# AndrewCullacino/handwritten-chinese-ocr-samples

Hardware: AMD Instinct MI355X
Metric: text-lines/sec (1x128x2000 synth) greedy decode (higher is better)
Workload: dtype f16 (f32 accumulate); 1 GPU; BASELINE configs[1]: 64 x 1x128x2000 uint8 lines, random-init hctr checkpoint (C=7358), forward + greedy CTC decode, labels to host; global_lines=64, lines_per_gpu=64, width=2000, classes=7358, checkpoint=random, parallelism=batch-shard x1

## Files before the change

### handwritten-chinese-ocr-samples_amd/csrc/kernels.hip

```cpp
#include "kernels.h"

#include <algorithm>
#include <cstdlib>

namespace hctr {

typedef _Float16 f16x8 __attribute__((ext_vector_type(8)));
typedef float f32x4 __attribute__((ext_vector_type(4)));
typedef float f32x2 __attribute__((ext_vector_type(2)));
typedef _Float16 f16x2 __attribute__((ext_vector_type(2)));
typedef uint32_t u32x4 __attribute__((ext_vector_type(4)));
typedef void __attribute__((address_space(3))) * lptr_t;

__device__ __forceinline__ void glds16_asm(const char* gsrc, char* lds_dst) {
    const uint32_t lds = (uint32_t)(uintptr_t)((lptr_t)lds_dst);
    uint32_t keep;
    asm volatile("s_mov_b32 %0, m0\n\ts_mov_b32 m0, %2\n\ts_nop 0\n\tglobal_load_lds_dwordx4 %1, off\n\ts_mov_b32 m0, %0"
                 : "=&s"(keep)
                 : "v"(gsrc), "s"(lds)
                 : "memory");
}

template <int CTRL>
__device__ __forceinline__ float dpp_f32(float v) {
    return __builtin_bit_cast(float, __builtin_amdgcn_update_dpp(0, __builtin_bit_cast(int, v), CTRL, 0xF, 0xF, true));
}

__device__ __forceinline__ bool np_gt(float a, float b) { return a > b || (a != a && b == b); }
__device__ __forceinline__ bool np_eq(float a, float b) { return a == b || (a != a && b != b); }

__device__ __forceinline__ void glds16_asm_s(const char* sbase, uint32_t voff, char* lds_dst) {
    const uint32_t lds = (uint32_t)(uintptr_t)((lptr_t)lds_dst);
    uint32_t keep;
    asm volatile("s_mov_b32 %0, m0\n\ts_mov_b32 m0, %3\n\ts_nop 0\n\tglobal_load_lds_dwordx4 %1, %2\n\ts_mov_b32 m0, %0"
                 : "=&s"(keep)
                 : "v"(voff), "s"(sbase), "s"(lds)
                 : "memory");
}

__device__ __forceinline__ void glds16x4_asm_s(const char* s0, const char* s1, const char* s2, const char* s3, uint32_t voff,
                                               char* d0, char* d1, char* d2, char* d3) {
    const uint32_t l0 = (uint32_t)(uintptr_t)((lptr_t)d0), l1 = (uint32_t)(uintptr_t)((lptr_t)d1);
    const uint32_t l2 = (uint32_t)(uintptr_t)((lptr_t)d2), l3 = (uint32_t)(uintptr_t)((lptr_t)d3);
    uint32_t keep;
    asm volatile("s_mov_b32 %0, m0\n\t"
                 "s_mov_b32 m0, %6\n\ts_nop 0\n\tglobal_load_lds_dwordx4 %1, %2\n\t"
                 "s_mov_b32 m0, %7\n\ts_nop 0\n\tglobal_load_lds_dwordx4 %1, %3\n\t"
                 "s_mov_b32 m0, %8\n\ts_nop 0\n\tglobal_load_lds_dwordx4 %1, %4\n\t"
                 "s_mov_b32 m0, %9\n\ts_nop 0\n\tglobal_load_lds_dwordx4 %1, %5\n\t"
                 "s_mov_b32 m0, %0"
                 : "=&s"(keep)
                 : "v"(voff), "s"(s0), "s"(s1), "s"(s2), "s"(s3), "s"(l0), "s"(l1), "s"(l2), "s"(l3)
                 : "memory");
}

template <int LSTRIDE>
__device__ __forceinline__ void glds16x4v_asm_s(const char* sbase, uint32_t v0, uint32_t v1, uint32_t v2, uint32_t v3, char* d0) {
    const uint32_t l0 = (uint32_t)(uintptr_t)((lptr_t)d0);
    uint32_t keep;
    asm volatile("s_mov_b32 %0, m0\n\t"
                 "s_mov_b32 m0, %6\n\ts_nop 0\n\tglobal_load_lds_dwordx4 %1, %5\n\t"
                 "s_add_u32 m0, m0, %7\n\ts_nop 0\n\tglobal_load_lds_dwordx4 %2, %5\n\t"
                 "s_add_u32 m0, m0, %7\n\ts_nop 0\n\tglobal_load_lds_dwordx4 %3, %5\n\t"
                 "s_add_u32 m0, m0, %7\n\ts_nop 0\n\tglobal_load_lds_dwordx4 %4, %5\n\t"
                 "s_mov_b32 m0, %0"
                 : "=&s"(keep)
                 : "v"(v0), "v"(v1), "v"(v2), "v"(v3), "s"(sbase), "s"(l0), "i"(LSTRIDE)
                 : "memory", "scc");
}

__device__ __forceinline__ constexpr int acc_cout_offset(int j) { return (j >> 2) * 64 + ((j >> 1) & 1) * 32 + (j & 1) * 4; }

constexpr float kSeScaleFloor = 1e-12f;

template <int WN, int WM, int JT, bool LINEAR, bool SPLIT, bool PRIVATE_RED = false, bool BIAS_DONE = false,
          bool RESID_IN_ACC = false>
__device__ __forceinline__ void conv_epilogue(const ConvArgs& a, f32x4 (&acc)[JT][4], char* smem, int tid, int lane,
                                              int wn, int wm, int n0, int mt, int img, int th, int tw, int hbase,
                                              int w0, unsigned long long* st = nullptr) {
    auto estamp = [&](int i) {
        if (st != nullptr) {
            __builtin_amdgcn_sched_barrier(0);
            if (tid == 0) st[i] = __builtin_amdgcn_s_memrealtime();
            __builtin_amdgcn_sched_barrier(0);
        }
    };
    constexpr int WC = JT * 16;
    constexpr int BN = WN * WC, BM = WM * 64;
    const int q = lane >> 4;
    const int c = lane & 15;
    const int cw0 = n0 + wn * WC + q * 8;
    auto co = [](int j) { return acc_cout_offset(j); };

    if (!BIAS_DONE) {
#pragma unroll
        for (int j = 0; j < JT; ++j) {
            const f32x4 b4 = *(const f32x4*)(a.bias + cw0 + co(j));
#pragma unroll
            for (int n = 0; n < 4; ++n)
#pragma unroll
                for (int i = 0; i < 4; ++i) acc[j][n][i] += b4[i];
        }
    }

    estamp(8);
    if (LINEAR && a.emit_cnt != nullptr) {
        static_assert(!LINEAR || WN == kLinearWN, "partials per n-tile");
        const int64_t part = (int64_t)((n0 / BN) * WN + wn) * a.M;
#pragma unroll
        for (int n = 0; n < 4; ++n) {
            const int64_t m = (int64_t)mt * BM + wm * 64 + n * 16 + c;
            const bool mv = m < a.M;
            const float vmin = mv ? a.row_thr[2 * m] : INFINITY;
            const float gmax = mv ? a.row_thr[2 * m + 1] : 0.f;
            double es = 0.0;
#pragma unroll
            for (int j = 0; j < JT; ++j)
#pragma unroll
                for (int i = 0; i < 4; ++i) {
                    const int cls = cw0 + co(j) + i;
                    const float v = acc[j][n][i];
                    if (cls < a.Cout) {
                        es += (double)expf(v - gmax);
                        if (v >= vmin) {
                            const int pos = atomicAdd(a.emit_cnt + m, 1);
                            if (pos < a.emit_cap) {
                                int32_t* e = a.emit_list + ((int64_t)m * a.emit_cap + pos) * 2;
                                e[0] = cls;
                                e[1] = __builtin_bit_cast(int32_t, v);
                            }
                        }
                    }
                }
            es += __shfl_xor(es, 16);
            es += __shfl_xor(es, 32);
            if (q == 0 && mv) a.esum[part + m] = es;
        }
        return;
    }
    if (LINEAR && a.amax_idx != nullptr) {
        static_assert(!LINEAR || WN == kLinearWN, "partials per n-tile");
        const int64_t part = (int64_t)((n0 / BN) * WN + wn) * a.M;
        const bool guard = a.amax_val2 != nullptr;
#pragma unroll
        for (int n = 0; n < 4; ++n) {
            float bv = -INFINITY, sv = -INFINITY, av = 0.f;
            int bi = 0x7fffffff;
            if (!guard) {
#pragma unroll
                for (int j = 0; j < JT; ++j)
#pragma unroll
                    for (int i = 0; i < 4; ++i) {
                        const int cls = cw0 + co(j) + i;
                        const float v = acc[j][n][i];
                        if (cls < a.Cout && np_gt(v, bv)) { bv = v; bi = cls; }
                    }
            } else {
#pragma unroll
                for (int j = 0; j < JT; ++j)
#pragma unroll
                    for (int i = 0; i < 4; ++i) {
                        const int cls = cw0 + co(j) + i;
                        const float v = acc[j][n][i];
                        if (cls < a.Cout) {
                            av = fmaxf(av, fabsf(v));
                            if (np_gt(v, bv)) { sv = bv; bv = v; bi = cls; }
                            else if (np_gt(v, sv)) sv = v;
                        }
                    }
            }
#pragma unroll
            for (int off = 16; off <= 32; off <<= 1) {
                const float ov = __shfl_xor(bv, off);
                const int oi = __shfl_xor(bi, off);
                const bool wins = np_gt(ov, bv) || (np_eq(ov, bv) && oi < bi);
                if (guard) {
                    const float osv = __shfl_xor(sv, off);
                    const float lose = wins ? bv : ov, keep2 = wins ? osv : sv;
                    sv = np_gt(lose, keep2) ? lose : keep2;
                    av = fmaxf(av, __shfl_xor(av, off));
                }
                if (wins) { bv = ov; bi = oi; }
            }
            const int64_t m = (int64_t)mt * BM + wm * 64 + n * 16 + c;
            if (q == 0 && m < a.M) {
                a.amax_val[part + m] = bv;
                a.amax_idx[part + m] = bi;
                if (guard) {
                    a.amax_val2[part + m] = sv;
                    a.amax_abs[part + m] = av;
                }
            }
            if (a.psum != nullptr) {
                float ps = 0.f;
#pragma unroll
                for (int j = 0; j < JT; ++j)
#pragma unroll
                    for (int i = 0; i < 4; ++i)
                        if (cw0 + co(j) + i < a.Cout) ps += expf(acc[j][n][i] - bv);
                ps += __shfl_xor(ps, 16);
                ps += __shfl_xor(ps, 32);
                if (q == 0 && m < a.M) {
                    a.psum[part + m] = ps;
                    if (cw0 == 0) a.blank_logit[m] = acc[0][n][0];
                }
            }
        }
        return;
    }
    if (LINEAR) {
        float* out = (float*)a.y;
#pragma unroll
        for (int n = 0; n < 4; ++n) {
            const int64_t m = (int64_t)mt * BM + wm * 64 + n * 16 + c;
            if (m < a.M) {
#pragma unroll
                for (int j = 0; j < JT; ++j)
                    *(f32x4*)(out + m * a.ldo + cw0 + co(j)) = acc[j][n];
            }
        }
        return;
    }

    const int w = w0 + c;
    const bool wvalid = w < a.W;
    half_t* out = (half_t*)a.y;
    const int64_t pix0 = a.out_off + img * a.out_sb + (int64_t)w * a.out_sw + cw0;

    if (SPLIT && !RESID_IN_ACC && a.se_scale != nullptr) {
        const float* sc = a.se_scale + (int64_t)img * a.Cout + cw0;
        if (w < a.out_wlimit) {
#pragma unroll
            for (int cb = 0; cb < JT / 4; ++cb)
#pragma unroll
                for (int n = 0; n < 4; ++n) {
                    const half_t* r = a.resid + pix0 + (int64_t)(hbase + n) * a.out_sh + cb * 64;
                    const f16x8 h0 = *(const f16x8*)r, h1 = *(const f16x8*)(r + 32);
                    const f16x8 l0 = *(const f16x8*)(r + a.Cout), l1 = *(const f16x8*)(r + a.Cout + 32);
#pragma unroll
                    for (int e = 0; e < 16; ++e) {
                        const float rv = e < 8 ? (float)h0[e] + (float)l0[e] : (float)h1[e - 8] + (float)l1[e - 8];
                        const float sv = sc[cb * 64 + (e >> 3) * 32 + (e & 7)];
                        acc[cb * 4 + (e >> 2)][n][e & 3] = fmaf(acc[cb * 4 + (e >> 2)][n][e & 3], sv, rv);
                    }
                }
        }
    } else if (RESID_IN_ACC) {
        const float* sc = a.se_scale + (int64_t)img * a.Cout + cw0;
#pragma unroll
        for (int j = 0; j < JT; ++j) {
            const f32x4 s4 = *(const f32x4*)(sc + co(j));
#pragma unroll
            for (int n = 0; n < 4; ++n)
#pragma unroll
                for (int i = 0; i < 4; ++i) acc[j][n][i] *= fmaxf(s4[i], kSeScaleFloor);
        }
    } else if (a.se_scale != nullptr) {
        const float* sc = a.se_scale + (int64_t)img * a.Cout + cw0;
        if (w < a.out_wlimit) {
            f16x8 rlo[JT / 4][4], rhi[JT / 4][4];
#pragma unroll
            for (int cb = 0; cb < JT / 4; ++cb)
#pragma unroll
                for (int n = 0; n < 4; ++n) {
                    const half_t* r = a.resid + pix0 + (int64_t)(hbase + n) * a.out_sh + cb * 64;
                    rlo[cb][n] = *(const f16x8*)r;
                    rhi[cb][n] = *(const f16x8*)(r + 32);
                }
#pragma unroll
            for (int j = 0; j < JT; ++j) {
                const f32x4 s4 = *(const f32x4*)(sc + co(j));
#pragma unroll
                for (int n = 0; n < 4; ++n)
#pragma unroll
                    for (int i = 0; i < 4; ++i) {
                        const int e = (j & 3) * 4 + i;
                        const float r = e < 8 ? (float)rlo[j >> 2][n][e] : (float)rhi[j >> 2][n][e - 8];
                        acc[j][n][i] = fmaf(acc[j][n][i], s4[i], r);
                    }
            }
        }
    }

    estamp(9);
    if (!SPLIT) {
        const _Float16 lo1 = a.relu ? (_Float16)0.f : (_Float16)(-INFINITY);
        const f16x2 lo2 = {lo1, lo1};
        const uint32_t keep = wvalid ? 0xffffffffu : 0u;
        uint32_t P[JT][4][2];
#pragma unroll
        for (int j = 0; j < JT; ++j)
#pragma unroll
            for (int n = 0; n < 4; ++n) {
                f32x4 v = acc[j][n];
                if (a.pool) {
                    const f32x4 u = acc[j][n | 1];
#pragma unroll
                    for (int i = 0; i < 4; ++i) v[i] = fmaxf(acc[j][n & ~1][i], u[i]);
                }
                f16x2 h0 = __builtin_convertvector((f32x2){v[0], v[1]}, f16x2);
                f16x2 h1 = __builtin_convertvector((f32x2){v[2], v[3]}, f16x2);
                h0 = __builtin_elementwise_max(h0, lo2);
                h1 = __builtin_elementwise_max(h1, lo2);
                P[j][n][0] = __builtin_bit_cast(uint32_t, h0) & keep;
                P[j][n][1] = __builtin_bit_cast(uint32_t, h1) & keep;
            }
        estamp(10);
        if (a.se_part != nullptr) {
            if (!PRIVATE_RED) {
                asm volatile("s_waitcnt vmcnt(0)" ::: "memory");
                __syncthreads();
            }
            float* red = (float*)smem;
            constexpr int NV = JT * 4;
            float vals[NV];
#pragma unroll
            for (int j = 0; j < JT; ++j)
#pragma unroll
                for (int i = 0; i < 4; ++i) {
                    float t[4];
#pragma unroll
                    for (int n = 0; n < 4; ++n)
                        t[n] = (float)__builtin_bit_cast(f16x2, P[j][n][i >> 1])[i & 1];
                    vals[j * 4 + i] = (t[0] + t[1]) + (t[2] + t[3]);
                }
            const bool e0 = ((c ^ (c >> 2)) & 1) != 0, e1 = (((c >> 1) ^ (c >> 2)) & 1) != 0;
            const bool e2 = (((c >> 2) ^ (c >> 3)) & 1) != 0, e3 = ((c >> 3) & 1) != 0;
            float r1[NV / 2], r2[NV / 4], r3[NV / 8], r4[NV / 16];
#pragma unroll
            for (int u = 0; u < NV / 2; ++u)
                r1[u] = (e0 ? vals[2 * u + 1] : vals[2 * u]) + dpp_f32<0xB1>(e0 ? vals[2 * u] : vals[2 * u + 1]);
#pragma unroll
            for (int u = 0; u < NV / 4; ++u)
                r2[u] = (e1 ? r1[2 * u + 1] : r1[2 * u]) + dpp_f32<0x4E>(e1 ? r1[2 * u] : r1[2 * u + 1]);
#pragma unroll
            for (int u = 0; u < NV / 8; ++u)
                r3[u] = (e2 ? r2[2 * u + 1] : r2[2 * u]) + dpp_f32<0x141>(e2 ? r2[2 * u] : r2[2 * u + 1]);
#pragma unroll
            for (int u = 0; u < NV / 16; ++u)
                r4[u] = (e3 ? r3[2 * u + 1] : r3[2 * u]) + dpp_f32<0x140>(e3 ? r3[2 * u] : r3[2 * u + 1]);
            const int vlow = (e3 ? 8 : 0) + (e2 ? 4 : 0) + (e1 ? 2 : 0) + (e0 ? 1 : 0);
#pragma unroll
            for (int u = 0; u < NV / 16; ++u) {
                const int v = 16 * u + vlow, j = v >> 2, i = v & 3;
                red[wm * BN + wn * WC + q * 8 + ((j >> 2) * 64 + ((j >> 1) & 1) * 32 + (j & 1) * 4) + i] = r4[u];
            }
            __syncthreads();
            if (tid < BN) {
                float sum = 0.f;
#pragma unroll
                for (int m = 0; m < WM; ++m) sum += red[m * BN + tid];
                const int64_t tile = (int64_t)img * (a.tilesH * a.tilesW) + th * a.tilesW + tw;
                if (n0 + tid < a.Cout) a.se_part[tile * a.Cout + n0 + tid] = sum;
            }
        }
        estamp(11);
        if (a.dbg & 256) {
            uint32_t t = 0;
#pragma unroll
            for (int j = 0; j < JT; ++j)
#pragma unroll
                for (int n = 0; n < 4; ++n) t += P[j][n][0] ^ P[j][n][1];
            if (t == 0x12345678u) out[0] = (half_t)1.f;
        } else if (w < a.out_wlimit) {
#pragma unroll
            for (int n = 0; n < 4; ++n) {
                if (a.pool && (n & 1)) continue;
                const int ho = a.pool ? ((hbase + n) >> 1) : (hbase + n);
                half_t* o = out + pix0 + (int64_t)ho * a.out_sh;
#pragma unroll
                for (int cb = 0; cb < JT / 4; ++cb) {
                    const int j0 = cb * 4;
                    *(u32x4*)(o + cb * 64) = (u32x4){P[j0][n][0], P[j0][n][1], P[j0 + 1][n][0], P[j0 + 1][n][1]};
                    *(u32x4*)(o + cb * 64 + 32) =
                        (u32x4){P[j0 + 2][n][0], P[j0 + 2][n][1], P[j0 + 3][n][0], P[j0 + 3][n][1]};
                }
            }
        }
        return;
    }
#pragma unroll
    for (int j = 0; j < JT; ++j)
#pragma unroll
        for (int n = 0; n < 4; ++n)
#pragma unroll
            for (int i = 0; i < 4; ++i) {
                float v = acc[j][n][i];
                if (a.pool && (n & 1) == 0) v = fmaxf(v, acc[j][n + 1][i]);
                if (a.relu) v = fmaxf(v, 0.f);
                if (!wvalid) v = 0.f;
                if (SPLIT) {
                    const half_t hi = (half_t)v;
                    v = a.drop_lo ? (float)hi : (float)hi + (float)(half_t)(v - (float)hi);
                } else {
                    v = (float)(half_t)v;
                }
                acc[j][n][i] = v;
            }

    estamp(10);
    if (a.se_part != nullptr) {
        if (!PRIVATE_RED) {
            asm volatile("s_waitcnt vmcnt(0)" ::: "memory");
            __syncthreads();
        }
        float* red = (float*)smem;
#pragma unroll
        for (int j = 0; j < JT; ++j)
#pragma unroll
            for (int i = 0; i < 4; ++i) {
                float s = (acc[j][0][i] + acc[j][1][i]) + (acc[j][2][i] + acc[j][3][i]);
                s += dpp_f32<0xB1>(s);
                s += dpp_f32<0x4E>(s);
                s += dpp_f32<0x141>(s);
                s += dpp_f32<0x140>(s);
                if (c == 0) red[wm * BN + wn * WC + q * 8 + co(j) + i] = s;
            }
        __syncthreads();
        if (tid < BN) {
            float s = 0.f;
#pragma unroll
            for (int m = 0; m < WM; ++m) s += red[m * BN + tid];
            const int64_t tile = (int64_t)img * (a.tilesH * a.tilesW) + th * a.tilesW + tw;
            if (n0 + tid < a.Cout) a.se_part[tile * a.Cout + n0 + tid] = s;
        }
    }

    estamp(11);
    if (a.dbg & 256) {
        float t = 0.f;
#pragma unroll
        for (int j = 0; j < JT; ++j)
#pragma unroll
            for (int n = 0; n < 4; ++n) t += acc[j][n][0] + acc[j][n][1] + acc[j][n][2] + acc[j][n][3];
        if (t == 123.456f) out[0] = (half_t)t;
    } else if (w < a.out_wlimit) {
#pragma unroll
        for (int n = 0; n < 4; ++n) {
            if (a.pool && (n & 1)) continue;
            const int ho = a.pool ? ((hbase + n) >> 1) : (hbase + n);
            half_t* o = out + pix0 + (int64_t)ho * a.out_sh;
#pragma unroll
            for (int cb = 0; cb < JT / 4; ++cb) {
                f16x8 lo, hi;
#pragma unroll
                for (int e = 0; e < 16; ++e) {
                    const half_t hv = (half_t)acc[cb * 4 + (e >> 2)][n][e & 3];
                    if (e < 8) lo[e] = hv; else hi[e - 8] = hv;
                }
                *(f16x8*)(o + cb * 64) = lo;
                *(f16x8*)(o + cb * 64 + 32) = hi;
                if (SPLIT) {
                    f16x8 l0, l1;
#pragma unroll
                    for (int e = 0; e < 16; ++e) {
                        const float v = acc[cb * 4 + (e >> 2)][n][e & 3];
                        const half_t lv = (half_t)(v - (float)(half_t)v);
                        if (e < 8) l0[e] = lv; else l1[e - 8] = lv;
                    }
                    *(f16x8*)(o + a.Cout + cb * 64) = l0;
                    *(f16x8*)(o + a.Cout + cb * 64 + 32) = l1;
                    *(f16x8*)(o + 2 * a.Cout + cb * 64) = lo;
                    *(f16x8*)(o + 2 * a.Cout + cb * 64 + 32) = hi;
                }
            }
        }
    }
}

template <int WN, int WM, int JT, int TAPS, bool LINEAR, bool PIPE, bool SPLIT>
__global__ __launch_bounds__(WN* WM * 64) void conv_mfma_kernel(const ConvArgs a) {
    constexpr int NT = WN * WM * 64;
    constexpr int WC = JT * 16;
    constexpr int BN = WN * WC, BM = WM * 64;
    constexpr int NIW = BN * 8 / NT;
    constexpr int NIX = BM * 8 / NT;
    constexpr int TILE_BYTES = (BN + BM) * 128;
    extern __shared__ __attribute__((aligned(16))) char smem[];

    const int tid = threadIdx.x;
    const int lane = tid & 63;
    const int wv = __builtin_amdgcn_readfirstlane(tid >> 6);
    const int wn = wv / WM, wm = wv % WM;

    const int total = a.mtiles * a.ntiles;
    int lin;
    {
        const int id = blockIdx.x, xcd = id & 7, s = id >> 3;
        const int q = total >> 3, r = total & 7;
        lin = (xcd < r ? xcd * (q + 1) : r * (q + 1) + (xcd - r) * q) + s;
    }
    const int nt = lin % a.ntiles;
    const int mt = lin / a.ntiles;
    const int n0 = nt * BN;

    int img = 0, th = 0, tw = 0;
    if (!LINEAR) {
        tw = mt % a.tilesW;
        const int t2 = mt / a.tilesW;
        th = t2 % a.tilesH;
        img = t2 / a.tilesH;
    }
    const int cin = a.Cin;

    const char* xbase;
    if (LINEAR) xbase = (const char*)(a.x + (int64_t)mt * BM * cin);
    else xbase = (const char*)(a.x + img * a.in_sb);
    const char* wbase = (const char*)(a.w + (int64_t)n0 * cin);
    uint32_t xoff[NIX], woff[NIW];
#pragma unroll
    for (int i = 0; i < NIX; ++i) {
        const int g = (wv * NIX + i) * 64 + lane;
        const int row = g >> 3, cp = (g & 7) ^ (row & 7);
        if (LINEAR) {
            int64_t rem = a.M - (int64_t)mt * BM;
            const int r = (int64_t)row < rem ? row : (int)rem - 1;
            xoff[i] = (uint32_t)r * (uint32_t)cin * 2u + cp * 16;
        } else {
            const int h = th * (4 * WM) + (row >> 6) * 4 + ((row >> 4) & 3);
            const int w = tw * kTileW + (row & 15);
            xoff[i] = ((uint32_t)(h + 1) * (uint32_t)a.in_sh + (uint32_t)(w + 1) * (uint32_t)cin) * 2u + cp * 16;
        }
    }
#pragma unroll
    for (int i = 0; i < NIW; ++i) {
        const int g = (wv * NIW + i) * 64 + lane;
        const int row = g >> 3, cp = (g & 7) ^ (row & 7);
        woff[i] = (uint32_t)row * (uint32_t)cin * 2u + cp * 16;
    }

    const int kc_steps = cin / kBK;
    const int nk = TAPS * kc_steps;

    auto step_offsets = [&](int k, int64_t& wo, int64_t& xo) {
        int tap = 0, kc = k;
        if (TAPS > 1) { kc = k / TAPS; tap = k - kc * TAPS; }
        xo = (int64_t)kc * (kBK * 2);
        if (TAPS > 1) {
            const int dy = tap / 3 - 1, dx = tap % 3 - 1;
            xo += ((int64_t)dy * a.in_sh + (int64_t)dx * cin) * 2;
        }
        wo = ((int64_t)tap * a.CoutPad * cin + (int64_t)kc * kBK) * 2;
    };
    auto stage_piece = [&](const char* wsrc, const char* xsrc, int buf, int idx) {
        if (idx < NIW) {
            char* wdst = smem + buf * TILE_BYTES + (wv * NIW) * 1024;
            glds16_asm_s(wsrc, woff[idx], wdst + idx * 1024);
        } else {
            char* xdst = smem + buf * TILE_BYTES + BN * 128 + (wv * NIX) * 1024;
            glds16_asm_s(xsrc, xoff[idx - NIW], xdst + (idx - NIW) * 1024);
        }
    };
    auto stage = [&](int k, int buf) {
        int64_t wo, xo;
        step_offsets(k, wo, xo);
#pragma unroll
        for (int i = 0; i < NIW + NIX; ++i) stage_piece(wbase + wo, xbase + xo, buf, i);
    };

    f32x4 acc[JT][4];
#pragma unroll
    for (int j = 0; j < JT; ++j)
#pragma unroll
        for (int n = 0; n < 4; ++n) acc[j][n] = (f32x4){0.f, 0.f, 0.f, 0.f};

    const int q = lane >> 4;
    const int frow = lane & 15;
    const int foff0 = frow * 128 + (((0 + q) ^ (lane & 7)) << 4);
    const int foff1 = frow * 128 + (((4 + q) ^ (lane & 7)) << 4);

    stage(0, 0);
    if (!PIPE) {
        for (int k = 0; k < nk; ++k) {
            asm volatile("s_waitcnt vmcnt(0)" ::: "memory");
            __syncthreads();
            const char* wt = smem + (k & 1) * TILE_BYTES + (wn * WC) * 128;
            const char* xt = smem + (k & 1) * TILE_BYTES + BN * 128 + (wm * 64) * 128;
            if (JT == 8) {
                f16x8 ar[3][2], bq[2][4];
                auto read_a = [&](int g, f16x8 (&dst)[2]) {
                    const char* base = wt + ((g >> 2) ? foff1 : foff0);
                    dst[0] = *(const f16x8*)(base + (2 * (g & 3)) * 2048);
                    dst[1] = *(const f16x8*)(base + (2 * (g & 3) + 1) * 2048);
                };
                auto read_b = [&](int ks, f16x8 (&dst)[4]) {
#pragma unroll
                    for (int n = 0; n < 4; ++n) dst[n] = *(const f16x8*)(xt + n * 2048 + (ks ? foff1 : foff0));
                };
                __builtin_amdgcn_sched_barrier(0);
                read_b(0, bq[0]);
                read_a(0, ar[0]);
                __builtin_amdgcn_sched_barrier(0);
                read_a(1, ar[1]);
                __builtin_amdgcn_sched_barrier(0);
                if (k + 1 < nk) stage(k + 1, (k + 1) & 1);
                __builtin_amdgcn_sched_barrier(0);
#pragma unroll
                for (int g = 0; g < 8; ++g) {
                    if (g + 2 < 8) read_a(g + 2, ar[(g + 2) % 3]);
                    __builtin_amdgcn_sched_barrier(0);
                    if (g == 1) { read_b(1, bq[1]); __builtin_amdgcn_sched_barrier(0); }
                    __builtin_amdgcn_s_setprio(1);
#pragma unroll
                    for (int jj = 0; jj < 2; ++jj)
#pragma unroll
                        for (int n = 0; n < 4; ++n)
                            acc[2 * (g & 3) + jj][n] = __builtin_amdgcn_mfma_f32_16x16x32_f16(ar[g % 3][jj], bq[g >> 2][n],
                                                                                             acc[2 * (g & 3) + jj][n], 0, 0, 0);
                    __builtin_amdgcn_s_setprio(0);
                    __builtin_amdgcn_sched_barrier(0);
                }
                continue;
            }
            if (k + 1 < nk) stage(k + 1, (k + 1) & 1);
#pragma unroll
            for (int ks = 0; ks < 2; ++ks) {
                const int fo = ks ? foff1 : foff0;
                f16x8 af[JT], bf[4];
#pragma unroll
                for (int n = 0; n < 4; ++n) bf[n] = *(const f16x8*)(xt + n * 2048 + fo);
#pragma unroll
                for (int j = 0; j < JT; ++j) af[j] = *(const f16x8*)(wt + j * 2048 + fo);
                __builtin_amdgcn_s_setprio(1);
#pragma unroll
                for (int j = 0; j < JT; ++j)
#pragma unroll
                    for (int n = 0; n < 4; ++n)
                        acc[j][n] = __builtin_amdgcn_mfma_f32_16x16x32_f16(af[j], bf[n], acc[j][n], 0, 0, 0);
                __builtin_amdgcn_s_setprio(0);
            }
        }
    } else {
        constexpr int NG = 2 * JT;
        constexpr int NP = NIW + NIX;
        for (int k = 0; k < nk; ++k) {
            asm volatile("s_waitcnt vmcnt(0)" ::: "memory");
            __syncthreads();
            const int kn = k + 1 < nk ? k + 1 : k;
            int64_t wo_n, xo_n;
            step_offsets(kn, wo_n, xo_n);
            const char* wsrc_n = wbase + wo_n;
            const char* xsrc_n = xbase + xo_n;
            const int buf_n = (k + 1) & 1;
            const char* wt = smem + (k & 1) * TILE_BYTES + (wn * WC) * 128;
            const char* xt = smem + (k & 1) * TILE_BYTES + BN * 128 + (wm * 64) * 128;
            f16x8 bfr[2][4], afr[2];
#pragma unroll
            for (int n = 0; n < 4; ++n) bfr[0][n] = *(const f16x8*)(xt + n * 2048 + foff0);
            afr[0] = *(const f16x8*)(wt + foff0);
#pragma unroll
            for (int g = 0; g < NG; ++g) {
                const int ks = g / JT, j = g % JT;
                if (g + 1 < NG) {
                    const int ks1 = (g + 1) / JT, j1 = (g + 1) % JT;
                    afr[(g + 1) & 1] = *(const f16x8*)(wt + j1 * 2048 + (ks1 ? foff1 : foff0));
                }
                if (g == JT / 2) {
#pragma unroll
                    for (int n = 0; n < 4; ++n) bfr[1][n] = *(const f16x8*)(xt + n * 2048 + foff1);
                }
                if ((g * NP) / NG != ((g + 1) * NP) / NG)
                    stage_piece(wsrc_n, xsrc_n, buf_n, (g * NP) / NG);
#pragma unroll
                for (int n = 0; n < 4; ++n)
                    acc[j][n] = __builtin_amdgcn_mfma_f32_16x16x32_f16(afr[g & 1], bfr[ks][n], acc[j][n], 0, 0, 0);
                __builtin_amdgcn_sched_barrier(0);
            }
        }
    }

    conv_epilogue<WN, WM, JT, LINEAR, SPLIT>(a, acc, smem, tid, lane, wn, wm, n0, mt, img, th, tw,
                                             th * (4 * WM) + wm * 4, tw * kTileW);
}

static int env_dbg() {
    if (getenv("HCTR_DBG_LAYER")) return 0;
    const char* e = getenv("HCTR_DBG");
    return e ? atoi(e) : 0;
}

static hipError_t raise_lds_limit(const void* fn, int bytes, bool (&done)[64]) {
    int dev = 0;
    hipError_t e = hipGetDevice(&dev);
// ... 3662 lines not shown
```

Measured before the change: 515.2 lines/s.

## Pipeline conv epilogue per channel-group with interleaved stores and SE partial reductions

Restructures the non-split conv epilogue so SE scaling/residual, pooling, f16 packing, output stores and the SE partial-sum DPP reduction run group by group over channel pairs, instead of in separate full passes. Scale loads for the next group are prefetched under sched barriers, and an interior-tile fast path drops the width masking. The __syncthreads calls become explicit waitcnt+s_barrier. The aim is to overlap stores with compute and cut register pressure from holding the whole packed tile, at the cost of more complex scheduling and a changed debug path.

Result: no change. 519.8 lines/s (median of 6 runs) (+0.9%).

```diff
diff --git a/handwritten-chinese-ocr-samples_amd/csrc/kernels.hip b/handwritten-chinese-ocr-samples_amd/csrc/kernels.hip
--- a/handwritten-chinese-ocr-samples_amd/csrc/kernels.hip
+++ b/handwritten-chinese-ocr-samples_amd/csrc/kernels.hip
@@ -245,7 +245,7 @@
                     }
                 }
         }
-    } else if (RESID_IN_ACC) {
+    } else if (SPLIT && RESID_IN_ACC) {
         const float* sc = a.se_scale + (int64_t)img * a.Cout + cw0;
 #pragma unroll
         for (int j = 0; j < JT; ++j) {
@@ -255,97 +255,149 @@
 #pragma unroll
                 for (int i = 0; i < 4; ++i) acc[j][n][i] *= fmaxf(s4[i], kSeScaleFloor);
         }
-    } else if (a.se_scale != nullptr) {
-        const float* sc = a.se_scale + (int64_t)img * a.Cout + cw0;
-        if (w < a.out_wlimit) {
-            f16x8 rlo[JT / 4][4], rhi[JT / 4][4];
-#pragma unroll
-            for (int cb = 0; cb < JT / 4; ++cb)
-#pragma unroll
-                for (int n = 0; n < 4; ++n) {
-                    const half_t* r = a.resid + pix0 + (int64_t)(hbase + n) * a.out_sh + cb * 64;
-                    rlo[cb][n] = *(const f16x8*)r;
-                    rhi[cb][n] = *(const f16x8*)(r + 32);
-                }
-#pragma unroll
-            for (int j = 0; j < JT; ++j) {
-                const f32x4 s4 = *(const f32x4*)(sc + co(j));
-#pragma unroll
-                for (int n = 0; n < 4; ++n)
-#pragma unroll
-                    for (int i = 0; i < 4; ++i) {
-                        const int e = (j & 3) * 4 + i;
-                        const float r = e < 8 ? (float)rlo[j >> 2][n][e] : (float)rhi[j >> 2][n][e - 8];
-                        acc[j][n][i] = fmaf(acc[j][n][i], s4[i], r);
-                    }
-            }
-        }
-    }
-
-    estamp(9);
+    }
+
     if (!SPLIT) {
+        static_assert(JT % 4 == 0, "groups pair up inside a 64-cout block");
         const _Float16 lo1 = a.relu ? (_Float16)0.f : (_Float16)(-INFINITY);
         const f16x2 lo2 = {lo1, lo1};
-        const uint32_t keep = wvalid ? 0xffffffffu : 0u;
-        uint32_t P[JT][4][2];
-#pragma unroll
-        for (int j = 0; j < JT; ++j)
-#pragma unroll
-            for (int n = 0; n < 4; ++n) {
-                f32x4 v = acc[j][n];
+        const bool se_sums = a.se_part != nullptr;
+        constexpr int NV = JT * 4;
+        const bool e0 = ((c ^ (c >> 2)) & 1) != 0, e1 = (((c >> 1) ^ (c >> 2)) & 1) != 0;
+        const bool e2 = (((c >> 2) ^ (c >> 3)) & 1) != 0, e3 = ((c >> 3) & 1) != 0;
+        float r3[NV / 8], r4[NV / 16];
+
+        auto pipeline = [&](auto edge_c) {
+            constexpr bool EDGE = decltype(edge_c)::value;
+            const bool in_limit = !EDGE || w < a.out_wlimit;
+            const bool st_ok = !EDGE || (w < a.out_wlimit && !(a.dbg & 256));
+            const uint32_t keep = wvalid ? 0xffffffffu : 0u;
+            const bool resid = !RESID_IN_ACC && a.se_scale != nullptr;
+            f32x4 s4[JT];
+            f16x8 rres[JT / 2][4];
+            const bool scaled = RESID_IN_ACC || (resid && in_limit);
+            const float* sc = a.se_scale + (int64_t)img * a.Cout + cw0;
+            auto load_scales = [&](int g) {
+                s4[2 * g] = *(const f32x4*)(sc + co(2 * g));
+                s4[2 * g + 1] = *(const f32x4*)(sc + co(2 * g + 1));
+            };
+            if (scaled) {
+                load_scales(0);
+                if (!RESID_IN_ACC) {
+#pragma unroll
+                    for (int g = 0; g < JT / 2; ++g)
+#pragma unroll
+                        for (int n = 0; n < 4; ++n)
+                            rres[g][n] = *(const f16x8*)(a.resid + pix0 + (int64_t)(hbase + n) * a.out_sh + co(2 * g));
+                }
+            }
+            if (!PRIVATE_RED && se_sums) {
+                asm volatile("s_waitcnt vmcnt(0)" ::: "memory");
+            }
+            __builtin_amdgcn_sched_barrier(0);
+#pragma unroll
+            for (int g = 0; g < JT / 2; ++g) {
+                const int j0 = 2 * g;
+                if (RESID_IN_ACC) {
+#pragma unroll
+                    for (int jj = 0; jj < 2; ++jj)
+#pragma unroll
+                        for (int n = 0; n < 4; ++n)
+#pragma unroll
+                            for (int i = 0; i < 4; ++i) acc[j0 + jj][n][i] *= fmaxf(s4[j0 + jj][i], kSeScaleFloor);
+                } else if (scaled) {
+#pragma unroll
+                    for (int jj = 0; jj < 2; ++jj)
+#pragma unroll
+                        for (int n = 0; n < 4; ++n)
+#pragma unroll
+                            for (int i = 0; i < 4; ++i)
+                                acc[j0 + jj][n][i] = fmaf(acc[j0 + jj][n][i], s4[j0 + jj][i], (float)rres[g][n][jj * 4 + i]);
+                }
+                if (g + 1 < JT / 2) {
+                    __builtin_amdgcn_sched_barrier(0);
+                    if (scaled) load_scales(g + 1);
+                }
                 if (a.pool) {
-                    const f32x4 u = acc[j][n | 1];
-#pragma unroll
-                    for (int i = 0; i < 4; ++i) v[i] = fmaxf(acc[j][n & ~1][i], u[i]);
-                }
-                f16x2 h0 = __builtin_convertvector((f32x2){v[0], v[1]}, f16x2);
-                f16x2 h1 = __builtin_convertvector((f32x2){v[2], v[3]}, f16x2);
-                h0 = __builtin_elementwise_max(h0, lo2);
-                h1 = __builtin_elementwise_max(h1, lo2);
-                P[j][n][0] = __builtin_bit_cast(uint32_t, h0) & keep;
-                P[j][n][1] = __builtin_bit_cast(uint32_t, h1) & keep;
-            }
-        estamp(10);
-        if (a.se_part != nullptr) {
-            if (!PRIVATE_RED) {
-                asm volatile("s_waitcnt vmcnt(0)" ::: "memory");
-                __syncthreads();
-            }
+#pragma unroll
+                    for (int jj = 0; jj < 2; ++jj)
+#pragma unroll
+                        for (int n = 0; n < 4; n += 2)
+#pragma unroll
+                            for (int i = 0; i < 4; ++i)
+                                acc[j0 + jj][n][i] = acc[j0 + jj][n + 1][i] = fmaxf(acc[j0 + jj][n][i], acc[j0 + jj][n + 1][i]);
+                }
+                uint32_t P[2][4][2];
+#pragma unroll
+                for (int n = 0; n < 4; ++n) {
+#pragma unroll
+                    for (int jj = 0; jj < 2; ++jj) {
+                        const int j = j0 + jj;
+                        const f32x4 v = acc[j][n];
+                        f16x2 h0 = __builtin_convertvector((f32x2){v[0], v[1]}, f16x2);
+                        f16x2 h1 = __builtin_convertvector((f32x2){v[2], v[3]}, f16x2);
+                        h0 = __builtin_elementwise_max(h0, lo2);
+                        h1 = __builtin_elementwise_max(h1, lo2);
+                        P[jj][n][0] = __builtin_bit_cast(uint32_t, h0);
+                        P[jj][n][1] = __builtin_bit_cast(uint32_t, h1);
+                        if (EDGE) {
+                            P[jj][n][0] &= keep;
+                            P[jj][n][1] &= keep;
+                        }
+                    }
+                    {
+                        const int ho = a.pool ? ((hbase + n) >> 1) : (hbase + n);
+                        half_t* o = out + pix0 + (int64_t)ho * a.out_sh + co(j0);
+                        if (st_ok && !((n & 1) && a.pool)) *(u32x4*)o = (u32x4){P[0][n][0], P[0][n][1], P[1][n][0], P[1][n][1]};
+                    }
+                    __builtin_amdgcn_sched_barrier(0);
+                    if (g == 0 && n == 0) estamp(9);
+                }
+                if (g == JT / 2 - 1) estamp(10);
+                if (se_sums) {
+                    float vals[8], r1[4], r2[2];
+#pragma unroll
+                    for (int jj = 0; jj < 2; ++jj)
+#pragma unroll
+                        for (int i = 0; i < 4; ++i) {
+                            float t[4];
+#pragma unroll
+                            for (int n = 0; n < 4; ++n)
+                                t[n] = (float)__builtin_bit_cast(f16x2, P[jj][n][i >> 1])[i & 1];
+                            vals[jj * 4 + i] = (t[0] + t[1]) + (t[2] + t[3]);
+                        }
+#pragma unroll
+                    for (int u = 0; u < 4; ++u)
+                        r1[u] = (e0 ? vals[2 * u + 1] : vals[2 * u]) + dpp_f32<0xB1>(e0 ? vals[2 * u] : vals[2 * u + 1]);
+#pragma unroll
+                    for (int u = 0; u < 2; ++u)
+                        r2[u] = (e1 ? r1[2 * u + 1] : r1[2 * u]) + dpp_f32<0x4E>(e1 ? r1[2 * u] : r1[2 * u + 1]);
+                    r3[g] = (e2 ? r2[1] : r2[0]) + dpp_f32<0x141>(e2 ? r2[0] : r2[1]);
+                    if (g & 1) r4[g >> 1] = (e3 ? r3[g] : r3[g - 1]) + dpp_f32<0x140>(e3 ? r3[g - 1] : r3[g]);
+                    __builtin_amdgcn_sched_barrier(0);
+                }
+            }
+        };
+        const int w0u = __builtin_amdgcn_readfirstlane(w0);
+        if (!(a.dbg & 256) && w0u + 16 <= a.W && w0u + 16 <= a.out_wlimit) pipeline(std::false_type{});
+        else pipeline(std::true_type{});
+
+        if (se_sums) {
+            auto lds_barrier = [] {
+                asm volatile("" ::: "memory");
+                __builtin_amdgcn_s_waitcnt(0xc07f);
+                __builtin_amdgcn_s_barrier();
+                asm volatile("" ::: "memory");
+            };
+            if (!PRIVATE_RED) lds_barrier();
             float* red = (float*)smem;
-            constexpr int NV = JT * 4;
-            float vals[NV];
-#pragma unroll
-            for (int j = 0; j < JT; ++j)
-#pragma unroll
-                for (int i = 0; i < 4; ++i) {
-                    float t[4];
-#pragma unroll
-                    for (int n = 0; n < 4; ++n)
-                        t[n] = (float)__builtin_bit_cast(f16x2, P[j][n][i >> 1])[i & 1];
-                    vals[j * 4 + i] = (t[0] + t[1]) + (t[2] + t[3]);
-                }
-            const bool e0 = ((c ^ (c >> 2)) & 1) != 0, e1 = (((c >> 1) ^ (c >> 2)) & 1) != 0;
-            const bool e2 = (((c >> 2) ^ (c >> 3)) & 1) != 0, e3 = ((c >> 3) & 1) != 0;
-            float r1[NV / 2], r2[NV / 4], r3[NV / 8], r4[NV / 16];
-#pragma unroll
-            for (int u = 0; u < NV / 2; ++u)
-                r1[u] = (e0 ? vals[2 * u + 1] : vals[2 * u]) + dpp_f32<0xB1>(e0 ? vals[2 * u] : vals[2 * u + 1]);
-#pragma unroll
-            for (int u = 0; u < NV / 4; ++u)
-                r2[u] = (e1 ? r1[2 * u + 1] : r1[2 * u]) + dpp_f32<0x4E>(e1 ? r1[2 * u] : r1[2 * u + 1]);
-#pragma unroll
-            for (int u = 0; u < NV / 8; ++u)
-                r3[u] = (e2 ? r2[2 * u + 1] : r2[2 * u]) + dpp_f32<0x141>(e2 ? r2[2 * u] : r2[2 * u + 1]);
-#pragma unroll
-            for (int u = 0; u < NV / 16; ++u)
-                r4[u] = (e3 ? r3[2 * u + 1] : r3[2 * u]) + dpp_f32<0x140>(e3 ? r3[2 * u] : r3[2 * u + 1]);
             const int vlow = (e3 ? 8 : 0) + (e2 ? 4 : 0) + (e1 ? 2 : 0) + (e0 ? 1 : 0);
 #pragma unroll
             for (int u = 0; u < NV / 16; ++u) {
                 const int v = 16 * u + vlow, j = v >> 2, i = v & 3;
                 red[wm * BN + wn * WC + q * 8 + ((j >> 2) * 64 + ((j >> 1) & 1) * 32 + (j & 1) * 4) + i] = r4[u];
             }
-            __syncthreads();
+            lds_barrier();
             if (tid < BN) {
                 float sum = 0.f;
 #pragma unroll
@@ -355,30 +407,9 @@
             }
         }
         estamp(11);
-        if (a.dbg & 256) {
-            uint32_t t = 0;
-#pragma unroll
-            for (int j = 0; j < JT; ++j)
-#pragma unroll
-                for (int n = 0; n < 4; ++n) t += P[j][n][0] ^ P[j][n][1];
-            if (t == 0x12345678u) out[0] = (half_t)1.f;
-        } else if (w < a.out_wlimit) {
-#pragma unroll
-            for (int n = 0; n < 4; ++n) {
-                if (a.pool && (n & 1)) continue;
-                const int ho = a.pool ? ((hbase + n) >> 1) : (hbase + n);
-                half_t* o = out + pix0 + (int64_t)ho * a.out_sh;
-#pragma unroll
-                for (int cb = 0; cb < JT / 4; ++cb) {
-                    const int j0 = cb * 4;
-                    *(u32x4*)(o + cb * 64) = (u32x4){P[j0][n][0], P[j0][n][1], P[j0 + 1][n][0], P[j0 + 1][n][1]};
-                    *(u32x4*)(o + cb * 64 + 32) =
-                        (u32x4){P[j0 + 2][n][0], P[j0 + 2][n][1], P[j0 + 3][n][0], P[j0 + 3][n][1]};
-                }
-            }
-        }
         return;
     }
+    estamp(9);
 #pragma unroll
     for (int j = 0; j < JT; ++j)
 #pragma unroll
```
